# afalchetti/monorfs

Measured on AMD Instinct MI355X. Metric: PHD updates/sec (particles x components x measurements), higher is better.
Workload: dtype f64; 1 GPU; RB-PHD-SLAM SlamUpdate, BASELINE config B: 2048 particles/GPU x 512 components x 64 measurements, PRM3D pixel-range model, prior weights 'survey', state resident in HBM; particles_per_gpu=2048, components=512, measurements=64, max_quantity=600, parallelism=particles sharded x1

## Files before the change

monorfs_amd/csrc/phd_sweep.h:

```cpp
#pragma once
#include "phd_device.h"

#ifndef SW_FIRST1
#define SW_FIRST1 128
#endif
#ifndef SW_TILE1
#define SW_TILE1  128
#endif
#define SW_REC    20
#define SW_UMAX   16

template <int ZB>
struct SweepLds {
	static constexpr int MP = ZB * 64;
	static constexpr int T = (ZB == 1) ? SW_TILE1 : 128;
	static constexpr int NMAP = 256 - T;
	static constexpr int MAPEACH = T / NMAP;
	static_assert(T % 64 == 0 && T < 256 && T % NMAP == 0, "tile: whole waves, and the map-space threads share it evenly");
	static constexpr int TD = (T * SW_REC > MP * 13) ? T * SW_REC : MP * 13;
	static constexpr int zs = 0, zmap = zs + 3 * MP, part = zmap + 3 * MP, part2 = part + 4 * MP, tile = part2 + 4 * MP,
	                     etab = tile + TD, du = etab + EXPTAB_N, ints = du + SW_UMAX;
	static constexpr int doubles = ints + (MP + SW_UMAX + 4) / 2;
};

template <int ZB, bool HALF = false, bool DEPTH = false>
__device__ __forceinline__ void sweep_body(const DevParams& prm, const StepBufs& a, double* pool)
{
	static_assert(!HALF || ZB == 1, "HALF is a layout of the one-block kernel");
	using L = SweepLds<ZB>;
	constexpr int MP = L::MP;
	double* const zs = pool + L::zs;
	double* const zmap = pool + L::zmap;
	double* const part = pool + L::part;
	double* const part2 = pool + L::part2;
	double* const tile = pool + L::tile;
	double* const etab = pool + L::etab;
	double* const s_du = pool + L::du;
	int* const born = (int*) (pool + L::ints);
	int* const s_ulist = born + MP;
	int& s_nb = born[MP + SW_UMAX];
	int& s_nmis = born[MP + SW_UMAX + 1];
	int& s_nu = born[MP + SW_UMAX + 2];

	const int p = a.p0 + blockIdx.x, tid = threadIdx.x, lane = tid & 63, wv = tid >> 6;
	const int M = a.M;
#ifdef PHD_STAMPS
	const long long st_c0 = clock64(), st_r0 = wall_clock64();
	long long st_pairc = 0, st_pairr = 0;
#endif
	const int klane = HALF ? (lane & 31) : lane;
	const int hoff  = HALF ? 4 * (lane >> 5) : 0;
	const bool owner = !HALF || lane < 32;
	const MixView vin = bank_view(a, SEL_IN);
	const Bank bin = bank_of(a, SEL_IN);
	const int n = vin.count[p];
	const size_t sb = in_base(a, p);
	const Bank bout = bank_of(a, SEL_OUT);
	PoseD pose = load_pose(bin.poses + (size_t) p * 7);
	pose.t[0] = uniform_d(pose.t[0]); pose.t[1] = uniform_d(pose.t[1]); pose.t[2] = uniform_d(pose.t[2]);
	pose.qw = uniform_d(pose.qw); pose.qx = uniform_d(pose.qx); pose.qy = uniform_d(pose.qy); pose.qz = uniform_d(pose.qz);
	if (tid < 7) bout.poses[(size_t) p * 7 + tid] = bin.poses[(size_t) p * 7 + tid];
	if (tid == 7) bout.weights[p] = bin.weights[p];
	auto rotation = [&](double* rq) {
		PoseD pq = pose;
		asm volatile("" : "+s"(pq.qw), "+s"(pq.qx), "+s"(pq.qy), "+s"(pq.qz));
		conj_matrix(pq, rq);
	};
	exp_tab_init(etab, tid);
	if (tid == 0) { s_nb = 0; s_nmis = 0; s_nu = 0; }
	for (int k = tid; k < MP; k += 256) {
		double z[3] = {0, 0, 1}, x[3] = {0, 0, 0};
		if (k < M) {
			z[0] = a.z[k * 3]; z[1] = a.z[k * 3 + 1]; z[2] = a.z[k * 3 + 2];
			measure_to_map(prm, pose, z, x);
		}
		zs[k * 3] = z[0]; zs[k * 3 + 1] = z[1]; zs[k * 3 + 2] = z[2];
		zmap[k * 3] = x[0]; zmap[k * 3 + 1] = x[1]; zmap[k * 3 + 2] = x[2];
	}
	__syncthreads();
	double zx[ZB], zy[ZB], zr[ZB], wx[ZB], wy[ZB], wz[ZB], wsum[ZB], dens[ZB];
	bool   zv[ZB];
#pragma unroll
	for (int b = 0; b < ZB; b++) {
		zv[b] = b * 64 + klane < M;
		wsum[b] = 0; dens[b] = 0;
	}
	auto load_z = [&]() {
#pragma unroll
		for (int b = 0; b < ZB; b++) {
			const int k = b * 64 + klane;
			zx[b] = zs[k * 3]; zy[b] = zs[k * 3 + 1]; zr[b] = zs[k * 3 + 2];
			wx[b] = zmap[k * 3]; wy[b] = zmap[k * 3 + 1]; wz[b] = zmap[k * 3 + 2];
		}
	};
	const double g2c = prm.g2_correct, g2e = prm.g2_explore, thr = prm.expl_thr;
	const int segcap = a.candcap >> 2;
	int2* cands = (int2*) a.cand + (size_t) p * a.candcap + (size_t) wv * segcap;
	int ncand_w = 0;

	const double cfac = prm.minw * 0.6065306597126334, ckap = cfac * prm.kappa;
	unsigned long long zvm[ZB];
#pragma unroll
	for (int b = 0; b < ZB; b++) zvm[b] = ballot64(zv[b]);
	const bool allpairs = a.all_pairs != 0;
	auto weigh = [&](const double* tt, int b, double sq, int c, bool cval) {
		const unsigned long long nm = ballot64(sq <= g2c) & (HALF ? ballot64(zv[b] && cval) : zvm[b]);
		if (nm || allpairs) {
			const double x = gauss_logw(tt, zx[b] - tt[0], zy[b] - tt[1], zr[b] - tt[2]);
			const double v = exp_pair(x, etab, zv[b] && sq <= g2c && (!HALF || cval));
			wsum[b] += v;
			const unsigned long long bal = ballot64(v >= fma(cfac, wsum[b], ckap)) & nm;
			if (bal) {
				if ((bal >> lane) & 1ull) {
					const int slot = ncand_w + __popcll(bal & lanemask_lt());
					if (slot < segcap) cands[slot] = make_int2((c << 8) | (b * 64 + klane), __float_as_int((float) x));
				}
				ncand_w += __popcll(bal);
			}
		}
	};

	auto sumk = [&](const double* arr, int k) {
		const double lo = arr[k] + arr[MP + k] + arr[2 * MP + k] + arr[3 * MP + k];
		if (!HALF) return lo;
		return lo + (arr[k + 32] + arr[MP + k + 32] + arr[2 * MP + k + 32] + arr[3 * MP + k + 32]);
	};

	bool compact = false;
	constexpr int SW_TILE = L::T, SW_NMAP = L::NMAP, SW_MAPEACH = L::MAPEACH;
	constexpr int SW_FIRST = (ZB == 1 && SW_FIRST1 < SW_TILE) ? SW_FIRST1 : SW_TILE;
	for (int c0 = 0, tl = SW_FIRST; c0 < n; c0 += tl, tl = SW_TILE) {
		{
			if (tid < SW_NMAP) {
#pragma unroll
				for (int q = 0; q < SW_MAPEACH; q++) {
					const int cl = tid + q * SW_NMAP, c = c0 + cl;
					if (c < n && cl < tl) {
						double P[6], m[3], Pi[6], det, w;
						load_comp(vin.rec + (sb + c) * MIX_REC, w, m, P);
						inv_sym3(P, Pi, det);
						gauss_record(w, m, Pi, PHD_INV_2PI / sqrt(fabs(det)), tile + cl * SW_REC + 10);
					}
				}
			}
			else {
				const int cl = tid - SW_NMAP, c = c0 + cl;
				bool mis = false;
				double wm = 0;
				if (c < n && cl < tl) {
					double* tt = tile + cl * SW_REC;
					double P[6], m[3], w;
					load_comp(vin.rec + (sb + c) * MIX_REC, w, m, P);
					CompMeas q;
					double rq[9];
					rotation(rq);
					comp_measure<DEPTH>(prm, pose, rq, m, P, q);
					tt[0] = q.zh[0]; tt[1] = q.zh[1]; tt[2] = q.zh[2];
					tt[3] = -0.5 * q.Sinv[0];
					tt[4] = -0.5 * (q.Sinv[1] + q.Sinv[3]);
					tt[5] = -0.5 * (q.Sinv[2] + q.Sinv[6]);
					tt[6] = -0.5 * q.Sinv[4];
					tt[7] = -0.5 * (q.Sinv[5] + q.Sinv[7]);
					tt[8] = -0.5 * q.Sinv[8];
					tt[9] = log(q.pd * w * q.qmult);
					wm  = (1 - q.pd) * w;
					mis = !(wm < prm.minw);
				}
				unsigned long long bal = ballot64(mis);
				if (bal) {
					int base = 0, first = __ffsll((long long) bal) - 1;
					if (lane == first) base = atomicAdd(&s_nmis, __popcll(bal));
					base = __shfl(base, first, 64);
					if (mis) {
						int slot = base + __popcll(bal & lanemask_lt());
						if (slot < a.ecap) {
							size_t e = (size_t) p * a.ecap + slot;
							a.emit_w[e]   = wm;
							a.emit_idx[e] = c;
						}
					}
				}
			}
		}
		__syncthreads();
		load_z();
		const int cend = min(tl, n - c0);
		if (compact) {
			const int nu = s_nu;
			for (int u = wv; u < nu; u += 4) {
				const int k = s_ulist[u];
				const double ux = zmap[k * 3], uy = zmap[k * 3 + 1], uz = zmap[k * 3 + 2];
				double acc = 0;
				for (int cc = lane; cc < cend; cc += 64) {
					const double* tt = tile + cc * SW_REC;
					const double e0 = ux - tt[10], e1 = uy - tt[11], e2 = uz - tt[12];
					const double vm = exp_neg(gauss_logw(tt + 10, e0, e1, e2), etab);
					if (e0 * e0 + e1 * e1 + e2 * e2 <= g2e) acc += vm;
				}
#pragma unroll
				for (int o = 32; o > 0; o >>= 1) acc += __shfl_xor(acc, o, 64);
				if (lane == 0) s_du[u] += acc;
			}
		}
		auto visit = [&](int cc) {
			const int ccl = HALF ? min(cc + hoff, cend - 1) : cc;
			const bool cval = !HALF || cc + hoff < cend;
			const double* tt = tile + ccl * SW_REC;
#pragma unroll
			for (int b = 0; b < ZB; b++) {
				double e0 = wx[b] - tt[10], e1 = wy[b] - tt[11], e2 = wz[b] - tt[12];
				double sq = e0 * e0 + e1 * e1 + e2 * e2;
				if (!compact && (allpairs || ballot64(sq <= g2e))) {
					double vm = exp_neg(gauss_logw(tt + 10, e0, e1, e2), etab);
					if (zv[b] && sq <= g2e && cval) dens[b] += vm;
				}
				weigh(tt, b, sq, c0 + ccl, cval);
			}
		};
		int cc = wv;
#ifdef PHD_STAMPS
		const long long st_pc = clock64(), st_pr = wall_clock64();
#endif
		if (HALF) {
			for (; cc < cend; cc += 8) visit(cc);
		}
		else {
			for (; cc + 4 < cend; cc += 8) { visit(cc); visit(cc + 4); }
			if (cc < cend) visit(cc);
		}
#ifdef PHD_STAMPS
		st_pairc += clock64() - st_pc; st_pairr += wall_clock64() - st_pr;
#endif
		if (!compact) {
#pragma unroll
			for (int b = 0; b < ZB; b++) part2[wv * MP + b * 64 + lane] = dens[b];
		}
		__syncthreads();
		if (!compact) {
			int nopen = 0;
			unsigned long long open[ZB];
#pragma unroll
			for (int b = 0; b < ZB; b++) {
				const int k = b * 64 + klane;
				const double d = sumk(part2, k);
				open[b] = ballot64(zv[b] && owner && !(d >= thr));
				nopen += __popcll(open[b]);
			}
			if (nopen <= SW_UMAX) {
				compact = true;
				if (wv == 0) {
					int base = 0;
#pragma unroll
					for (int b = 0; b < ZB; b++) {
						if ((open[b] >> lane) & 1ull) {
							const int u = base + __popcll(open[b] & lanemask_lt());
							s_ulist[u] = b * 64 + lane;
							s_du[u] = 0.0;
						}
						base += __popcll(open[b]);
					}
					if (lane == 0) s_nu = nopen;
				}
			}
		}
	}

#pragma unroll
	for (int b = 0; b < ZB; b++) part2[wv * MP + b * 64 + lane] = dens[b];
	__syncthreads();
	for (int k = tid; k < MP; k += 256) {
		double d = (k < M) ? sumk(part2, k) : 0.0;
		born[k] = (k < M) && !(d >= thr);
	}
	__syncthreads();
	if (tid < s_nu) {
		const int k = s_ulist[tid];
		const double d = sumk(part2, k) + s_du[tid];
		born[k] = !(d >= thr);
	}
	__syncthreads();
	if (tid == 0) {
		int nb = 0;
		for (int k = 0; k < M; k++) {
			if (born[k]) {
				a.born_k[(size_t) p * a.Mcap + nb] = k;
				a.born_mean[((size_t) p * a.Mcap + nb) * 3]     = zmap[k * 3];
				a.born_mean[((size_t) p * a.Mcap + nb) * 3 + 1] = zmap[k * 3 + 1];
				a.born_mean[((size_t) p * a.Mcap + nb) * 3 + 2] = zmap[k * 3 + 2];
				born[nb] = k;
				nb++;
			}
		}
		a.born_count[p] = nb;
		s_nb = nb;
	}
	__syncthreads();
	const int nb = s_nb;
	const int nmis0 = s_nmis;
	__syncthreads();
	if (tid == 0) s_nmis = 0;
	__syncthreads();
	{
		for (int b0 = 0; b0 < nb; b0 += 256) {
			const int bi = b0 + tid;
			bool mis = false;
			double wm = 0, m[3] = {0, 0, 0};
			if (bi < nb) {
				const int k = born[bi];
				m[0] = zmap[k * 3]; m[1] = zmap[k * 3 + 1]; m[2] = zmap[k * 3 + 2];
				CompMeas q;
				double rq[9];
				rotation(rq);
				comp_measure<DEPTH>(prm, pose, rq, m, prm.birthP, q);
				double* tt = tile + bi * 13;
				tt[0] = q.zh[0]; tt[1] = q.zh[1]; tt[2] = q.zh[2];
				tt[3] = -0.5 * q.Sinv[0];
				tt[4] = -0.5 * (q.Sinv[1] + q.Sinv[3]);
				tt[5] = -0.5 * (q.Sinv[2] + q.Sinv[6]);
				tt[6] = -0.5 * q.Sinv[4];
				tt[7] = -0.5 * (q.Sinv[5] + q.Sinv[7]);
				tt[8] = -0.5 * q.Sinv[8];
				tt[9] = log(q.pd * prm.birthw * q.qmult);
				tt[10] = m[0]; tt[11] = m[1]; tt[12] = m[2];
				wm  = (1 - q.pd) * prm.birthw;
				mis = !(wm < prm.minw);
			}
			unsigned long long bal = ballot64(mis);
			if (bal) {
				int base = 0, first = __ffsll((long long) bal) - 1;
				if (lane == first) base = atomicAdd(&s_nmis, __popcll(bal));
				base = __shfl(base, first, 64);
				if (mis) {
					int slot = nmis0 + base + __popcll(bal & lanemask_lt());
					if (slot < a.ecap) {
						size_t e = (size_t) p * a.ecap + slot;
						a.emit_w[e]   = wm;
						a.emit_idx[e] = n + bi;
					}
				}
			}
		}
	}
	__syncthreads();
	load_z();
	for (int bi = (wv - n) & 3; bi < nb; bi += HALF ? 8 : 4) {
		const int bil = HALF ? min(bi + hoff, nb - 1) : bi;
		const bool cval = !HALF || bi + hoff < nb;
		const double* tt = tile + bil * 13;
#pragma unroll
		for (int b = 0; b < ZB; b++) {
			double e0 = wx[b] - tt[10], e1 = wy[b] - tt[11], e2 = wz[b] - tt[12];
			weigh(tt, b, e0 * e0 + e1 * e1 + e2 * e2, n + bil, cval);
		}
	}
#pragma unroll
	for (int b = 0; b < ZB; b++) part[wv * MP + b * 64 + lane] = wsum[b];
	__syncthreads();
	for (int k = tid; k < M; k += 256) {
		a.denom[(size_t) p * a.Mcap + k] = prm.kappa + sumk(part, k);
	}
	if (lane == 0) a.cand_count[(size_t) p * 4 + wv] = ncand_w;
	if (tid == 0) {
		int ne = nmis0 + s_nmis;
		if (ne > a.ecap) { atomicOr(a.flags, PHD_FLAG_EMIT_OVERFLOW); ne = a.ecap; }
		a.emit_count[p] = ne;
	}
#ifdef PHD_STAMPS
	if (tid == 0 && a.stamps && a.stamp_kernel == 6) {
		double* o = a.stamps + (size_t) p * 16;
		o[0] = 0; o[1] = (double) (clock64() - st_c0); o[2] = (double) (wall_clock64() - st_r0); o[3] = (double) st_pairc; o[4] = (double) st_pairr;
	}
#endif
}

#ifndef PHD_SWEEP_WAVES
#define PHD_SWEEP_WAVES 4
#endif
template <int ZB, bool HALF = false, bool DEPTH = false>
#ifndef PHD_SWEEP2_WAVES
#define PHD_SWEEP2_WAVES PHD_SWEEP_WAVES
#endif
__global__ __launch_bounds__(256, (ZB == 4 ? 2 : (ZB == 2 ? PHD_SWEEP2_WAVES : PHD_SWEEP_WAVES))) void k_sweep(const DevParams prm, const StepBufs a)
{
	__shared__ __align__(16) double pool[SweepLds<ZB>::doubles];
	PHD_TL_BEGIN;
	PHD_SET_PRIO(PHD_DENSE_PRIO);
	sweep_body<ZB, HALF, DEPTH>(prm, a, pool);
	PHD_TL_END(6);
}
```

monorfs_amd/csrc/phd_alpha.h:

```cpp
#pragma once
#include "phd_device.h"


__device__ __forceinline__ int pk_get(unsigned int perm, int i) { return (int) ((perm >> (4 * i)) & 15u); }

__device__ __forceinline__ unsigned int pk_set(unsigned int perm, int i, int v)
{
	return (perm & ~(15u << (4 * i))) | ((unsigned int) v << (4 * i));
}

__device__ __forceinline__ unsigned int pk_reverse(unsigned int perm, int from, int to)
{
	for (int i = from, j = to - 1; i < j; i++, j--) {
		int vi = pk_get(perm, i), vj = pk_get(perm, j);
		perm = pk_set(pk_set(perm, i, vj), j, vi);
	}
	return perm;
}

__device__ __forceinline__ bool pk_last(unsigned int perm, int n)
{
	for (int i = 1; i < n; i++) {
		if (pk_get(perm, i - 1) < pk_get(perm, i)) return false;
	}
// ... 682 lines not shown
	__syncthreads();
	const double r = red[0];
	__syncthreads();
	return r;
}

template <int MW>
__device__ __forceinline__ bool has_detection(const unsigned long long* adj, int j)
{
	bool has = false;
#pragma unroll
	for (int b = 0; b < MW; b++) has |= adj[(size_t) j * MW + b] != 0;
	return has;
}

template <int ZB, bool QUASI, bool GRAD = false, int TAG = 0, bool DEPTH = false>
__device__ __forceinline__ void alpha_assoc_body(const DevParams& prm, const StepBufs& a, int ncap, double* smem, double* gws = nullptr,
                                                 int* helper_go = nullptr)
{
	constexpr int MP = ZB * 64;
	constexpr int MW = ZB;
	constexpr int JL = ALPHA_JL;
	const AlphaLds lay = alpha_lds(MP, ncap);
	double* zs   = smem + lay.zs;
	double* red  = smem + lay.red;
	double* etab = red;
	__shared__ int s_J, s_changed[2], s_nroots, s_big;
	__shared__ double s_ccount, s_total;
	__shared__ int s_ebump, s_g2lds;
	__shared__ double s_g2[GRAD ? QGRAD_G2_CLUSTERS * QGRAD_HDR + QGRAD_G2_WEIGHTS : 2];
	if (GRAD && threadIdx.x == 0) s_g2lds = 0;

	const int p = a.p0 + blockIdx.x, tid = threadIdx.x, lane = tid & 63, wv = tid >> 6;
	const int M = a.M, cap = a.cap;
	const MixView vout = bank_view(a, SEL_OUT);
	const Bank bin = bank_of(a, SEL_IN);
	const int no = QUASI ? 0 : vout.count[p];
	const size_t sbo = (size_t) p * cap;
	const PoseD pose = load_pose(QUASI ? a.qposes + (size_t) p * 7 : bin.poses + (size_t) p * 7);

	for (int k = tid; k < MP * 3; k += 256) zs[k] = (k < M * 3) ? a.z[k] : 0.0;
	unsigned int helper_word = 0;
	if (!QUASI && helper_go && tid == 0) helper_word = __hip_atomic_load(a.dsync + 3 * (size_t) p, __ATOMIC_RELAXED, __HIP_MEMORY_SCOPE_AGENT);

	PHD_STAMP_DECL;
	PHD_STAMP(0);
	double* keyw    = smem + lay.p1_keyw;
	double* sortw   = smem + lay.p1_sortw;
	int*    sortsrc = (int*) (smem + lay.p1_sortsrc);
	auto block_sum = [&](double v) { return block_tree_sum(red, v, tid); };
	double wpart = 0;
	for (int c = tid; c < no; c += 256) {
		double wc = a.outw[sbo + c];
		keyw[c] = wc;
		wpart += wc;
	}
	{
		double e = block_sum(wpart);
		if (fabs(e - rint(e)) <= 1e-9 * fmax(1.0, fabs(e))) {
			if (tid == 0) {
				double q = 0;
				for (int c = 0; c < no; c++) q += keyw[c];
				s_ccount = q;
			}
			__syncthreads();
			e = s_ccount;
		}
		if (tid == 0) {
			s_ccount = e;
			int J = (int) e;
			if (J < 0) J = 0;
			if (J > a.Jcap) {
				atomicOr(a.flags, PHD_FLAG_J_OVERFLOW);
				J = a.Jcap;
			}
			s_J = QUASI ? min(a.qJ, a.Jcap) : J;
		}
	}
	PHD_STAMP(1);
	__syncthreads();
	const int J = s_J;
	if (J >= 1 && J <= no) {
		constexpr int HB = 500;
		int* const hist   = (int*) red;
		int* const selidx = (int*) (smem + lay.p1_selidx);
		int* const pre    = (int*) (smem + lay.p1_dw);
		int& s_T = hist[HB];
		int& s_above = hist[HB + 1];
		int& s_nt = hist[HB + 2];
		const unsigned int hbase = (unsigned int) (((unsigned long long) __double_as_longlong(prm.minw) << 1) >> 49);
		auto bin_of = [&](double w) {
			const unsigned int k = (unsigned int) (((unsigned long long) __double_as_longlong(w) << 1) >> 49);
			return (int) min(max((int) k - (int) hbase, 0), HB - 1);
		};
		for (int t = tid; t < HB + 4; t += 256) hist[t] = 0;
		__syncthreads();
		for (int c = tid; c < no; c += 256) atomicAdd(&hist[bin_of(keyw[c])], 1);
		__syncthreads();
		if (wv == 0) {
			int cq[8], mine = 0;
#pragma unroll
			for (int q = 0; q < 8; q++) { const int b = 511 - (8 * lane + q); cq[q] = (b < HB) ? hist[b] : 0; mine += cq[q]; }
			int incl = mine;
#pragma unroll
			for (int o = 1; o < 64; o <<= 1) {
				const int y = __shfl_up(incl, o, 64);
				if (lane >= o) incl += y;
			}
			int run = incl - mine;
#pragma unroll
			for (int q = 0; q < 8; q++) {
				const int b = 511 - (8 * lane + q);
				if (b < HB) pre[b] = run;
				if (run < J && J <= run + cq[q]) { s_T = b; s_above = run; s_nt = cq[q]; }
				run += cq[q];
			}
		}
		__syncthreads();
		const int T = s_T, above = s_above;
		const int ncand = above + s_nt;
		for (int c = tid; c < no; c += 256) {
			const int b = bin_of(keyw[c]);
			if (b >= T) selidx[pre[b] + atomicSub(&hist[b], 1) - 1] = c;
		}
		__syncthreads();
		for (int e = tid; e < ncand; e += 256) {
			const int ce = selidx[e];
			const double we = keyw[ce];
			const int b = bin_of(we);
			const int lo = pre[b], hi = (b == T) ? ncand : pre[b - 1];
			int rank = lo;
#pragma unroll 4
			for (int u = lo; u < hi; u++) {
				const int cu = selidx[u];
				const double wu = keyw[cu];
				rank += (wu > we || (wu == we && cu < ce)) ? 1 : 0;
			}
			if (rank < J) { sortw[rank] = we; sortsrc[rank] = ce; }
		}
		__syncthreads();
	}
	else if (!QUASI && J > no) {
		unsigned long long* sv = (unsigned long long*) sortw;
		int NS = 2;
		while (NS < no) NS <<= 1;
		for (int t = tid; t < NS; t += 256) sv[t] = (t < no) ? prune_pack(keyw[t], t) : 0ull;
		__syncthreads();
		prune_bitonic(sv, NS, tid);
		for (int r = tid; r + 1 < no; r += 256) {
			const unsigned long long kb = prune_kbits(sv[r]);
			if (prune_kbits(sv[r + 1]) != kb || (r > 0 && prune_kbits(sv[r - 1]) == kb)) continue;
			int e = r + 2;
			while (e < no && prune_kbits(sv[e]) == kb) e++;
			for (int x = r + 1; x < e; x++) {
				unsigned long long vx = sv[x];
				int sx = prune_slot(vx);
				double wx = keyw[sx];
				int y = x - 1;
				while (y >= r) {
					int sy = prune_slot(sv[y]);
					if (keyw[sy] > wx || (keyw[sy] == wx && sy < sx)) break;
					sv[y + 1] = sv[y];
					y--;
				}
				sv[y + 1] = vx;
			}
		}
		__syncthreads();
		for (int r = tid; r < no; r += 256) sortsrc[r] = prune_slot(sv[r]);
		__syncthreads();
		for (int r = tid; r < no; r += 256) sortw[r] = keyw[sortsrc[r]];
		__syncthreads();
	}
	PHD_STAMP(2);
	const bool inlds = J <= JL;
	const int  JS = inlds ? JL : a.Jcap;
	double* gj = a.jscratch + (size_t) p * alpha_jscratch_doubles(a.Jcap);
	double* lm   = inlds ? smem + lay.lm     : gj + AlphaSlab::lm * (size_t) JS;
	double* dw   = inlds ? smem + lay.p1_dw  : gj + AlphaSlab::dw * (size_t) JS;
	double* zh   = inlds ? smem + lay.p3_zh  : gj + AlphaSlab::zh * (size_t) JS;
	double* lpd  = inlds ? smem + lay.p3_pdj : gj + AlphaSlab::lpd * (size_t) JS;
	double* lmd  = inlds ? smem + lay.p3_lmd : gj + AlphaSlab::lmd * (size_t) JS;
	double* res  = inlds ? smem + lay.p3_res : gj + AlphaSlab::res * (size_t) JS;
	unsigned long long* adj = (unsigned long long*) (inlds ? smem + lay.p3_adj : gj + AlphaSlab::adj * (size_t) JS);
	int* gi      = (int*) (gj + AlphaSlab::ints * (size_t) JS);
	int* pick    = inlds ? (int*) (smem + lay.pick) : gi + AlphaSlab::i_pick * JS;
	int* dsrc    = inlds ? sortsrc + lay.ns : gi + AlphaSlab::i_dsrc * JS;
	int* labl    = inlds ? (int*) (smem + lay.p3_int) : gi + AlphaSlab::i_labl * JS;
	int* roots   = inlds ? labl + JL : gi + AlphaSlab::i_roots * JS;
	int* cnt     = inlds ? labl + 2 * JL : (int*) (gj + AlphaSlab::cnt * (size_t) JS);
	unsigned long long* memL = (unsigned long long*) (inlds ? smem + lay.p3_mem : gj + AlphaSlab::memL * (size_t) JS);
	unsigned long long* memZ = (unsigned long long*) (inlds ? smem + lay.p3_mem + JL : gj + AlphaSlab::memZ * (size_t) JS);
	int* labz    = (int*) (smem + lay.p3_int) + 3 * JL;
	double* xreg = smem + lay.p3_x;
	const bool straight = J <= no && (J == 0 || !(sortw[0] - 1 > sortw[J - 1]));
	if (QUASI) {}
	else if (straight) {
		for (int j = tid; j < J; j += 256) pick[j] = sortsrc[j];
	}
	else if (tid == 0) {
		int ia = 0, id = 0, nd = 0;
		for (int j = 0; j < J; j++) {
			bool takeorig;
			if (ia < no && id < nd) takeorig = !(dw[id] > sortw[ia]);
			else takeorig = ia < no;
			double wpick;
			int    src;
			if (takeorig) { wpick = sortw[ia]; src = sortsrc[ia]; ia++; }
			else          { wpick = dw[id];    src = dsrc[id];    id++; }
			dw[nd]   = wpick - 1;
			dsrc[nd] = src;
			nd++;
			pick[j] = src;
		}
	}
	__threadfence_block();
	__syncthreads();
	constexpr int JW = JL / 64;
	unsigned long long* adjT = (unsigned long long*) (smem + lay.p3_adjT);
	for (int k = tid; k < M; k += 256) labz[k] = J + k;
	for (int t = tid; t < MP * JW; t += 256) adjT[t] = 0;
	if (tid == 0) { s_nroots = 0; s_big = 0; s_changed[0] = 0; }
	for (int j = tid; j < J; j += 256) {
		double2 r0 = {0.0, 0.0}, r1 = {0.0, 0.0};
		if (!QUASI) {
			const double2* rc = (const double2*) (vout.rec + (sbo + pick[j]) * MIX_REC);
			r0 = rc[0]; r1 = rc[1];
		}
#pragma unroll
		for (int b = 0; b < MW; b++) adj[(size_t) j * MW + b] = 0;
		labl[j] = j;
		cnt[j]  = 0;
		memL[j] = 0;
		memZ[j] = 0;
		if (QUASI) {
			lm[j] = a.qlm[j * 3]; lm[JS + j] = a.qlm[j * 3 + 1]; lm[2 * JS + j] = a.qlm[j * 3 + 2];
		}
		else {
			double l0 = r0.y, l1 = r1.x, l2 = r1.y;
			lm[j] = l0; lm[JS + j] = l1; lm[2 * JS + j] = l2;
			double* glm = a.alm + (size_t) p * 3 * a.Jcap;
			glm[j] = l0; glm[a.Jcap + j] = l1; glm[2 * a.Jcap + j] = l2;
		}
	}
	if (!QUASI && helper_go) {
		if (tid == 0) { a.aJ[p] = J; a.account[p] = s_ccount; }
		asm volatile("s_waitcnt vmcnt(0)" ::: "memory");
	}
	__threadfence_block();
	__syncthreads();
	if (!QUASI && helper_go && tid == 0) {
		const int go = (dens_layout(J) != DensLayout::slab && helper_word == ((a.dstamp << 4) | my_xcd())) ? 1 : 0;
		__hip_atomic_store(a.dsync + 3 * (size_t) p + 1, 2u * a.dstamp + (unsigned int) go, __ATOMIC_RELAXED, __HIP_MEMORY_SCOPE_AGENT);
		*helper_go = go;
#ifdef PHD_STAMPS
		if (a.stamps && a.stamp_kernel == 5) { a.stamps[(size_t) p * 16 + 12] = go; a.stamps[(size_t) p * 16 + 13] = (double) wall_clock64(); }
#endif
	}

	PHD_STAMP(3);
	{
		double* mats = xreg;

		const bool pair = J <= 128;
		for (int t = tid; t < (pair ? 256 : J); t += 256) {
			const int j = pair ? (t & 127) : t;
			if (j >= J) continue;
			double m[3] = {lm[j], lm[JS + j], lm[2 * JS + j]}, z[3], l[3];
			measure_perfect(prm, pose, m, z, l);
			const float dz = (!QUASI && DEPTH) ? depth_at(prm, z) : 0.0f;
			const double pdv = QUASI ? prm.pd : detection_probability_m<!QUASI && DEPTH>(prm, z, dz);
			if (!pair || t < 128) {
				zh[j] = z[0]; zh[JS + j] = z[1]; zh[2 * JS + j] = z[2];
				lpd[j] = log(pdv);
			}
			if (!pair || t >= 128) lmd[j] = log(1 - pdv);
		}
		__threadfence_block();
		__syncthreads();
		{
			double kx[ZB], ky[ZB], kz[ZB];
#pragma unroll
			for (int b = 0; b < ZB; b++) {
				const int k = b * 64 + lane;
				kx[b] = zs[k * 3]; ky[b] = zs[k * 3 + 1]; kz[b] = zs[k * 3 + 2];
			}
			const double g2 = QUASI ? prm.g2_quasi : prm.g2_assoc;
			for (int j = wv; j < J; j += 4) {
				const double h0 = zh[j], h1 = zh[JS + j], h2 = zh[2 * JS + j];
#pragma unroll
				for (int b = 0; b < ZB; b++) {
					const int k = b * 64 + lane;
					const bool gated = k < M && quad_gen(prm.Rinv, h0 - kx[b], h1 - ky[b], h2 - kz[b]) < g2;
					const unsigned long long bal = ballot64(gated);
					if (lane == 0) adj[(size_t) j * MW + b] = bal;
					if (gated && inlds) atomicOr(&adjT[(size_t) k * JW + (j >> 6)], 1ull << (j & 63));
				}
			}
		}
		__threadfence_block();
		__syncthreads();

		PHD_STAMP(4);
		for (int it = 0; it < J + M + 1; it++) {
			int* const changed = &s_changed[it & 1];
			for (int j = tid; j < J; j += 256) {
				int l = labl[j];
#pragma unroll
				for (int b = 0; b < MW; b++) {
					unsigned long long bits = adj[(size_t) j * MW + b];
					while (bits) {
						int k = b * 64 + __ffsll((long long) bits) - 1;
						bits &= bits - 1;
						l = min(l, labz[k]);
					}
				}
				if (l < labl[j]) { labl[j] = l; *changed = 1; }
			}
			__threadfence_block();
			__syncthreads();
			if (tid == 0) s_changed[(it & 1) ^ 1] = 0;
			for (int k = tid; k < M; k += 256) {
				int l = labz[k];
				if (inlds) {
#pragma unroll
					for (int b = 0; b < JW; b++) {
						unsigned long long bits = adjT[(size_t) k * JW + b];
						while (bits) {
							int j = b * 64 + __ffsll((long long) bits) - 1;
							bits &= bits - 1;
							l = min(l, labl[j]);
						}
					}
				}
				else {
					for (int j = 0; j < J; j++) {
						if ((adj[(size_t) j * MW + (k >> 6)] >> (k & 63)) & 1ull) l = min(l, labl[j]);
					}
				}
				if (l < labz[k]) { labz[k] = l; *changed = 1; }
			}
			__threadfence_block();
			__syncthreads();
			if (!*changed) break;
		}
		for (int j = tid; j < J; j += 256) {
			const int r = labl[j];
			const int slot = atomicAdd(&cnt[r], 1) & 0xffff;
			if (slot < 5) atomicOr(&memL[r], (unsigned long long) j << (12 * slot));
		}
		for (int k = tid; k < M; k += 256) {
			const int r = labz[k];
			if (r < J) {
				const int slot = atomicAdd(&cnt[r], 0x10000) >> 16;
				if (slot < 5) atomicOr(&memZ[r], (unsigned long long) k << (12 * slot));
			}
		}
		if (wv == 0) {
			int nr = 0;
			for (int j0 = 0; j0 < J; j0 += 64) {
				const int j = j0 + lane;
				bool isroot = false;
				if (j < J) {
					const bool has = has_detection<MW>(adj, j);
					isroot = has && labl[j] == j;
				}
				unsigned long long bal = ballot64(isroot);
				if (isroot) roots[nr + __popcll(bal & lanemask_lt())] = j;
				nr += __popcll(bal);
			}
			if (lane == 0) s_nroots = nr;
		}
		exp_tab_init(etab, tid);
		__syncthreads();
		const int nroots = s_nroots;
		const double logmult = prm.logRmult;

		PHD_STAMP(5);
		if (GRAD) {
			if (tid == 0) s_big = 1;
		}
		else if (J >= 5) {
			for (int ri = tid; ri < nroots; ri += 256) {
				const int root = roots[ri];
				const int cn = cnt[root];
				const int nl = cn & 0xffff, nz = cn >> 16;
				if (nl + nz > 5) {
					res[ri] = NAN;
					s_big = 1;
					continue;
				}
				const unsigned long long Lp = pk_sort5(memL[root], nl), Zp = pk_sort5(memZ[root], nz);
				double E[25];
#pragma unroll
				for (int e = 0; e < 25; e++) E[e] = (e % 6 == 0) ? 1.0 : 0.0;
				double rsum = 0;
				bool dead = false;
#pragma unroll
				for (int x = 0; x < 4; x++) {
					if (x < nl) {
						const int j = (int) ((Lp >> (12 * x)) & 4095);
						const double md = lmd[j], lp = lpd[j];
						const double h0 = zh[j], h1 = zh[JS + j], h2 = zh[2 * JS + j];
						double D[4], rx = md;
#pragma unroll
						for (int y = 0; y < 4 - x; y++) {
							D[y] = -INFINITY;
							if (y < nz) {
								const int k = (int) ((Zp >> (12 * y)) & 4095);
								if ((adj[(size_t) j * MW + (k >> 6)] >> (k & 63)) & 1ull) {
									double dist = sqrt(quad_gen(prm.Rinv, h0 - zs[k * 3], h1 - zs[k * 3 + 1], h2 - zs[k * 3 + 2]));
									D[y] = lp + logmult - 0.5 * dist * dist;
									rx = fmax(rx, D[y]);
								}
							}
						}
						if (rx == -INFINITY) dead = true;
						else {
							rsum += rx;
							E[x * 6] = exp_neg(md - rx, etab);
#pragma unroll
							for (int y = 0; y < 4 - x; y++) {
								if (y < nz) E[x * 5 + 4 - y] = (D[y] == -INFINITY) ? 0.0 : exp_neg(D[y] - rx, etab);
							}
						}
					}
				}
#pragma unroll
				for (int y = 0; y < 4; y++) {
					if (y < nz) {
						E[(4 - y) * 6] = prm.kappa;
#pragma unroll
						for (int x = 0; x < 4 - y; x++) {
							if (x < nl) E[(4 - y) * 5 + x] = 1.0;
						}
					}
				}
				double f[32];
#pragma unroll
				for (int m = 0; m < 32; m++) f[m] = 0;
				f[0] = 1;
#pragma unroll
				for (int i = 0; i < 5; i++) {
#pragma unroll
					for (int m = 0; m < 32; m++) {
						if (__builtin_popcount(m) == i) {
#pragma unroll
							for (int c = 0; c < 5; c++) {
								if (!((m >> c) & 1)) f[m | (1 << c)] = fma(f[m], E[i * 5 + c], f[m | (1 << c)]);
							}
						}
					}
				}
				res[ri] = dead ? -INFINITY : rsum + log(f[31]);
			}
		}
		else if (wv == 0) {
			for (int r0 = 0; r0 < nroots; r0 += 64) {
				int ri = r0 + lane;
				if (ri < nroots) {
					int root = roots[ri];
					unsigned long long Lp = 0, Zp = 0;
					int nl = 0, nz = 0, nrow = 0;
					for (int j = root; j < J; j++) {
						if (labl[j] == root) { if (nl < 5) Lp |= (unsigned long long) j << (12 * nl); nl++; }
					}
					for (int k = 0; k < M; k++) {
						if (labz[k] == root) { if (nz < 5) Zp |= (unsigned long long) k << (12 * nz); nz++; }
					}
					nrow = nl + nz;
					if (nrow > 5) {
						res[ri] = NAN;
						s_big = 1;
					}
					else {
						double* mat = mats + lane;
						for (int e = 0; e < 25; e++) mat[e * 4] = -INFINITY;
						for (int x = 0; x < nl; x++) {
							int j = (int) ((Lp >> (12 * x)) & 4095);
							for (int y = 0; y < nz; y++) {
								int k = (int) ((Zp >> (12 * y)) & 4095);
								if ((adj[(size_t) j * MW + (k >> 6)] >> (k & 63)) & 1ull) {
									double dist = sqrt(quad_gen(prm.Rinv, zh[j] - zs[k * 3], zh[JS + j] - zs[k * 3 + 1],
									                            zh[2 * JS + j] - zs[k * 3 + 2]));
									mat[(x * 5 + y) * 4] = lpd[j] + logmult - 0.5 * dist * dist;
								}
							}
							mat[(x * 5 + nz + x) * 4] = lmd[j];
						}
						for (int y = 0; y < nz; y++) {
							mat[((nl + y) * 5 + y) * 4] = prm.logkappa;
							for (int x = 0; x < nl; x++) mat[((nl + y) * 5 + nz + x) * 4] = 0;
						}
						res[ri] = cluster_enumerate(mat, 4, nrow, J);
					}
				}
			}
		}
		__syncthreads();
		if (GRAD && gws && inlds) {
			double* const wsm = gws + wv * QGRAD_WAVE_DOUBLES;
			double* const gmat = wsm;
			double* const gjp = wsm + 25;
			double (*gdv)[6] = (double (*)[6]) (wsm + 25 + 5 * 18);
			double* const glc = wsm + 25 + 5 * 18 + 120 * 6;
			int* const gL = (int*) (glc + 120);
			int* const gZ = gL + 8;
			double* const jpall = gj + AlphaSlab::g_jpall;
			double* const elist = gj + AlphaSlab::g_elist;
			const int ecap = (int) alpha_jscratch_doubles(a.Jcap) - AlphaSlab::g_elist;
			const int gt = (lane < 6) ? lane : 0;
			if (tid == 0) s_ebump = 0;
			if (ecap > 0) {
				for (int j = tid; j < J; j += 256) {
					const double m3[3] = {lm[j], lm[JS + j], lm[2 * JS + j]};
					jacobian_p(prm, pose, m3, jpall + (size_t) j * 18);
				}
			}
			__threadfence_block();
			__syncthreads();
			const bool pairfast = J >= 5 && ecap > 0;
			if (pairfast) {
				for (int ri = tid; ri < nroots; ri += 256) {
					const int root = roots[ri];
					if (cnt[root] != 0x10001) continue;
					const int j = (int) (memL[root] & 4095), k = (int) (memZ[root] & 4095);
					double* const h = gj + (size_t) ri * QGRAD_HDR;
					const bool gated = (adj[(size_t) j * MW + (k >> 6)] >> (k & 63)) & 1ull;
					double c0 = -INFINITY;
					if (gated) {
						double dist = sqrt(quad_gen(prm.Rinv, zh[j] - zs[k * 3], zh[JS + j] - zs[k * 3 + 1], zh[2 * JS + j] - zs[k * 3 + 2]));
						c0 = lpd[j] + logmult - 0.5 * dist * dist;
					}
					c0 = (0.0 + c0) + 0.0;
					const double c1 = (0.0 + lmd[j]) + prm.logkappa;
					const double mx = fmax(fmax(-INFINITY, c0), c1);
					const bool finite = !(isinf(mx) && mx < 0);
					double lse = -INFINITY, w0 = c0, w1 = c1;
					if (finite) {
						double value = 0;
						value += exp(c0 - mx);
						value += exp(c1 - mx);
						lse = mx + log(value);
						w0 = exp_neg(c0 - mx, etab);
						w1 = exp_neg(c1 - mx, etab);
					}
					res[ri] = lse;
					const int off = atomicAdd(&s_ebump, 2);
					if (off + 2 > ecap) { h[0] = -2; continue; }
					elist[off] = w0;
					elist[off + 1] = w1;
					double G[6] = {0, 0, 0, 0, 0, 0};
					if (finite && gated) {
						const double nu[3] = {zs[k * 3] - zh[j], zs[k * 3 + 1] - zh[JS + j], zs[k * 3 + 2] - zh[2 * JS + j]};
						const double* Jp = jpall + (size_t) j * 18;
#pragma unroll
						for (int t = 0; t < 6; t++) G[t] = w0 * (0.0 + pair_gradient(prm, nu, Jp, t));
					}
					h[0] = 2.0;
#pragma unroll
					for (int t = 0; t < 6; t++) h[1 + t] = G[t];
					h[7] = (double) off;
					h[8] = finite ? 1.0 : 0.0;
				}
			}
			PHD_STAMP(9);
			for (int ri = wv; ri < nroots; ri += 4) {
				const int root = roots[ri];
				if (pairfast && cnt[root] == 0x10001) continue;
				double* const h = gj + (size_t) ri * QGRAD_HDR;
				int nl = 0, nz = 0;
				for (int j0 = root; j0 < J; j0 += 64) {
					const int j = j0 + lane;
					const bool in = j < J && labl[j] == root;
					const unsigned long long bal = ballot64(in);
					const int pos = nl + __popcll(bal & lanemask_lt());
					if (in && pos < 6) gL[pos] = j;
					nl += __popcll(bal);
				}
				for (int k0 = 0; k0 < M; k0 += 64) {
					const int k = k0 + lane;
					const bool in = k < M && labz[k] == root;
					const unsigned long long bal = ballot64(in);
					const int pos = nz + __popcll(bal & lanemask_lt());
					if (in && pos < 6) gZ[pos] = k;
					nz += __popcll(bal);
				}
				const int nrow = nl + nz;
				if (nrow > 5) {
					if (lane == 0) h[0] = -1;
					continue;
				}
				lds_fence();
				if (lane < nrow * nrow) {
					const int x = lane / nrow, y = lane - x * nrow;
					double v = -INFINITY;
					if (x < nl) {
						const int j = gL[x];
						if (y < nz) {
							const int k = gZ[y];
							if ((adj[(size_t) j * MW + (k >> 6)] >> (k & 63)) & 1ull) {
								double dist = sqrt(quad_gen(prm.Rinv, zh[j] - zs[k * 3], zh[JS + j] - zs[k * 3 + 1], zh[2 * JS + j] - zs[k * 3 + 2]));
								v = lpd[j] + logmult - 0.5 * dist * dist;
							}
						}
						else if (y - nz == x) v = lmd[j];
					}
					else {
						if (y < nz) { if (y == x - nl) v = prm.logkappa; }
						else v = 0;
					}
					gmat[x * 5 + y] = v;
				}
				if (ecap <= 0) {
					if (lane == 0) h[0] = -2;
					continue;
				}
				int mcount;
				double mx = -INFINITY, value = 0;
				if (nrow <= J) {
					double* const pgt = gjp;
					const int npair = nl * nz;
					bool g = false;
					{
						const int pr = lane / 6, t = lane - 6 * pr;
						if (pr < npair) {
							const int x = pr / nz, y = pr - x * nz;
							const int j = gL[x], k = gZ[y];
							g = (adj[(size_t) j * MW + (k >> 6)] >> (k & 63)) & 1ull;
							double v = 0;
							if (g) {
								const double nu[3] = {zs[k * 3] - zh[j], zs[k * 3 + 1] - zh[JS + j], zs[k * 3 + 2] - zh[2 * JS + j]};
								v = pair_gradient(prm, nu, jpall + (size_t) j * 18, t);
							}
							pgt[(x * 4 + y) * 6 + t] = v;
						}
					}
					const unsigned long long gb = ballot64(g);
					unsigned int gmask = 0;
					for (int pr = 0; pr < npair; pr++) {
						if ((gb >> (6 * pr)) & 1ull) gmask |= 1u << ((pr / nz) * 4 + (pr % nz));
					}
					lds_fence();
					mcount = 1;
					for (int i = 2; i <= nrow; i++) mcount *= i;
					double vv[2] = {-INFINITY, -INFINITY};
#pragma unroll
					for (int pass = 0; pass < 2; pass++) {
						const int m = lane + 64 * pass;
						if (m < mcount) {
							const unsigned int perm = pk_unrank(m, nrow);
							double v = 0;
							for (int i = 0; i < nrow; i++) v += gmat[i * 5 + pk_get(perm, i)];
							double acc[6] = {0, 0, 0, 0, 0, 0};
							for (int x = 0; x < nl; x++) {
								const int y = pk_get(perm, x);
								if (y < nz && ((gmask >> (x * 4 + y)) & 1u)) {
#pragma unroll
									for (int t = 0; t < 6; t++) acc[t] += pgt[(x * 4 + y) * 6 + t];
								}
							}
							glc[m] = v;
#pragma unroll
							for (int t = 0; t < 6; t++) gdv[m][t] = acc[t];
							vv[pass] = v;
						}
					}
					mx = fmax(vv[0], vv[1]);
#pragma unroll
					for (int o = 32; o > 0; o >>= 1) mx = fmax(mx, __shfl_xor(mx, o, 64));
					if (!(isinf(mx) && mx < 0)) {
						const double e0 = (lane < mcount) ? exp(vv[0] - mx) : 0.0, e1 = (lane + 64 < mcount) ? exp(vv[1] - mx) : 0.0;
						auto rld = [](double v, int l) {
							return __hiloint2double(__builtin_amdgcn_readlane(__double2hiint(v), l), __builtin_amdgcn_readlane(__double2loint(v), l));
						};
						for (int i = 0; i < mcount; i++) value += (i < 64) ? rld(e0, i) : rld(e1, i - 64);
// ... 863 lines not shown
```

Before: 125.3 billion PHD updates/s.

## Build sweep birth list with wave ballots and drop serial scan and barriers

After: 125.9 billion PHD updates/s (median of 6 runs). About the same (+0.5%).

```diff
diff --git a/monorfs_amd/csrc/phd_sweep.h b/monorfs_amd/csrc/phd_sweep.h
--- a/monorfs_amd/csrc/phd_sweep.h
+++ b/monorfs_amd/csrc/phd_sweep.h
@@ -22,6 +22,8 @@
 	                     etab = tile + TD, du = etab + EXPTAB_N, ints = du + SW_UMAX;
 	static constexpr int doubles = ints + (MP + SW_UMAX + 4) / 2;
 };
+static_assert(SweepLds<1>::doubles * 8 <= 32768 && 4 * SweepLds<2>::doubles * 8 <= 160 * 1024,
+              "k_sweep<1> and k_sweep<2> run four workgroups per CU: their LDS must fit 160 KiB four times");
 
 template <int ZB, bool HALF = false, bool DEPTH = false>
 __device__ __forceinline__ void sweep_body(const DevParams& prm, const StepBufs& a, double* pool)
@@ -47,6 +49,8 @@
 #ifdef PHD_STAMPS
 	const long long st_c0 = clock64(), st_r0 = wall_clock64();
 	long long st_pairc = 0, st_pairr = 0;
+	long long st_tail = st_c0, st_list = 0, st_stage = 0;
+	int st_switch = -1, st_tile = 0;
 #endif
 	const int klane = HALF ? (lane & 31) : lane;
 	const int hoff  = HALF ? 4 * (lane >> 5) : 0;
@@ -65,6 +69,23 @@
 		PoseD pq = pose;
 		asm volatile("" : "+s"(pq.qw), "+s"(pq.qx), "+s"(pq.qy), "+s"(pq.qz));
 		conj_matrix(pq, rq);
+	};
+	auto birth_record = [&](int k, double* tt) {
+		const double m[3] = {zmap[k * 3], zmap[k * 3 + 1], zmap[k * 3 + 2]};
+		CompMeas q;
+		double rq[9];
+		rotation(rq);
+		comp_measure<DEPTH>(prm, pose, rq, m, prm.birthP, q);
+		tt[0] = q.zh[0]; tt[1] = q.zh[1]; tt[2] = q.zh[2];
+		tt[3] = -0.5 * q.Sinv[0];
+		tt[4] = -0.5 * (q.Sinv[1] + q.Sinv[3]);
+		tt[5] = -0.5 * (q.Sinv[2] + q.Sinv[6]);
+		tt[6] = -0.5 * q.Sinv[4];
+		tt[7] = -0.5 * (q.Sinv[5] + q.Sinv[7]);
+		tt[8] = -0.5 * q.Sinv[8];
+		tt[9] = log(q.pd * prm.birthw * q.qmult);
+		tt[10] = m[0]; tt[11] = m[1]; tt[12] = m[2];
+		return (1 - q.pd) * prm.birthw;
 	};
 	exp_tab_init(etab, tid);
 	if (tid == 0) { s_nb = 0; s_nmis = 0; s_nu = 0; }
@@ -230,6 +251,7 @@
 		}
 #ifdef PHD_STAMPS
 		st_pairc += clock64() - st_pc; st_pairr += wall_clock64() - st_pr;
+		st_tail = clock64();
 #endif
 		if (!compact) {
 #pragma unroll
@@ -248,6 +270,9 @@
 			}
 			if (nopen <= SW_UMAX) {
 				compact = true;
+#ifdef PHD_STAMPS
+				st_switch = st_tile;
+#endif
 				if (wv == 0) {
 					int base = 0;
 #pragma unroll
@@ -263,66 +288,78 @@
 				}
 			}
 		}
-	}
-
-#pragma unroll
-	for (int b = 0; b < ZB; b++) part2[wv * MP + b * 64 + lane] = dens[b];
+#ifdef PHD_STAMPS
+		st_tile++;
+#endif
+	}
+
+	if (n == 0) {
+#pragma unroll
+		for (int b = 0; b < ZB; b++) part2[wv * MP + b * 64 + lane] = dens[b];
+		__syncthreads();
+	}
+#ifdef PHD_STAMPS
+	st_list = clock64();
+#endif
+	if (wv == 0) {
+		int nbw = 0;
+		auto list = [&](bool isb, int k, int bi) {
+			if (isb) {
+				a.born_k[(size_t) p * a.Mcap + bi] = k;
+				a.born_mean[((size_t) p * a.Mcap + bi) * 3]     = zmap[k * 3];
+				a.born_mean[((size_t) p * a.Mcap + bi) * 3 + 1] = zmap[k * 3 + 1];
+				a.born_mean[((size_t) p * a.Mcap + bi) * 3 + 2] = zmap[k * 3 + 2];
+				born[bi] = k;
+			}
+		};
+		if (compact) {
+			const int nu = s_nu;
+			bool isb = false;
+			int k = 0;
+			if (lane < nu) {
+				k = s_ulist[lane];
+				const double d = sumk(part2, k) + s_du[lane];
+				isb = !(d >= thr);
+			}
+			const unsigned long long bal = ballot64(isb);
+			const int bi = __popcll(bal & lanemask_lt());
+			nbw = __popcll(bal);
+			list(isb, k, bi);
+		}
+		else {
+			bool isb[ZB];
+			unsigned long long bal[ZB];
+#pragma unroll
+			for (int b = 0; b < ZB; b++) {
+				const int k = b * 64 + lane;
+				const double d = (k < M) ? sumk(part2, k) : 0.0;
+				isb[b] = (k < M) && !(d >= thr);
+				bal[b] = ballot64(isb[b]);
+			}
+#pragma unroll
+			for (int b = 0; b < ZB; b++) {
+				list(isb[b], b * 64 + lane, nbw + __popcll(bal[b] & lanemask_lt()));
+				nbw += __popcll(bal[b]);
+			}
+		}
+		if (lane == 0) {
+			a.born_count[p] = nbw;
+			s_nb = nbw;
+		}
+	}
 	__syncthreads();
-	for (int k = tid; k < MP; k += 256) {
-		double d = (k < M) ? sumk(part2, k) : 0.0;
-		born[k] = (k < M) && !(d >= thr);
-	}
-	__syncthreads();
-	if (tid < s_nu) {
-		const int k = s_ulist[tid];
-		const double d = sumk(part2, k) + s_du[tid];
-		born[k] = !(d >= thr);
-	}
-	__syncthreads();
-	if (tid == 0) {
-		int nb = 0;
-		for (int k = 0; k < M; k++) {
-			if (born[k]) {
-				a.born_k[(size_t) p * a.Mcap + nb] = k;
-				a.born_mean[((size_t) p * a.Mcap + nb) * 3]     = zmap[k * 3];
-				a.born_mean[((size_t) p * a.Mcap + nb) * 3 + 1] = zmap[k * 3 + 1];
-				a.born_mean[((size_t) p * a.Mcap + nb) * 3 + 2] = zmap[k * 3 + 2];
-				born[nb] = k;
-				nb++;
-			}
-		}
-		a.born_count[p] = nb;
-		s_nb = nb;
-	}
-	__syncthreads();
-	const int nb = s_nb;
-	const int nmis0 = s_nmis;
-	__syncthreads();
-	if (tid == 0) s_nmis = 0;
-	__syncthreads();
-	{
+#ifdef PHD_STAMPS
+	st_stage = clock64();
+	st_list = st_stage - st_list;
+#endif
+	const int nb = __builtin_amdgcn_readfirstlane(s_nb);
+	if (nb > 0) {
 		for (int b0 = 0; b0 < nb; b0 += 256) {
 			const int bi = b0 + tid;
 			bool mis = false;
-			double wm = 0, m[3] = {0, 0, 0};
+			double wm = 0;
 			if (bi < nb) {
-				const int k = born[bi];
-				m[0] = zmap[k * 3]; m[1] = zmap[k * 3 + 1]; m[2] = zmap[k * 3 + 2];
-				CompMeas q;
-				double rq[9];
-				rotation(rq);
-				comp_measure<DEPTH>(prm, pose, rq, m, prm.birthP, q);
-				double* tt = tile + bi * 13;
-				tt[0] = q.zh[0]; tt[1] = q.zh[1]; tt[2] = q.zh[2];
-				tt[3] = -0.5 * q.Sinv[0];
-				tt[4] = -0.5 * (q.Sinv[1] + q.Sinv[3]);
-				tt[5] = -0.5 * (q.Sinv[2] + q.Sinv[6]);
-				tt[6] = -0.5 * q.Sinv[4];
-				tt[7] = -0.5 * (q.Sinv[5] + q.Sinv[7]);
-				tt[8] = -0.5 * q.Sinv[8];
-				tt[9] = log(q.pd * prm.birthw * q.qmult);
-				tt[10] = m[0]; tt[11] = m[1]; tt[12] = m[2];
-				wm  = (1 - q.pd) * prm.birthw;
+				wm  = birth_record(born[bi], tile + bi * 13);
 				mis = !(wm < prm.minw);
 			}
 			unsigned long long bal = ballot64(mis);
@@ -331,7 +368,7 @@
 				if (lane == first) base = atomicAdd(&s_nmis, __popcll(bal));
 				base = __shfl(base, first, 64);
 				if (mis) {
-					int slot = nmis0 + base + __popcll(bal & lanemask_lt());
+					int slot = base + __popcll(bal & lanemask_lt());
 					if (slot < a.ecap) {
 						size_t e = (size_t) p * a.ecap + slot;
 						a.emit_w[e]   = wm;
@@ -340,8 +377,11 @@
 				}
 			}
 		}
-	}
-	__syncthreads();
+		__syncthreads();
+	}
+#ifdef PHD_STAMPS
+	st_stage = clock64() - st_stage;
+#endif
 	load_z();
 	for (int bi = (wv - n) & 3; bi < nb; bi += HALF ? 8 : 4) {
 		const int bil = HALF ? min(bi + hoff, nb - 1) : bi;
@@ -361,7 +401,7 @@
 	}
 	if (lane == 0) a.cand_count[(size_t) p * 4 + wv] = ncand_w;
 	if (tid == 0) {
-		int ne = nmis0 + s_nmis;
+		int ne = s_nmis;
 		if (ne > a.ecap) { atomicOr(a.flags, PHD_FLAG_EMIT_OVERFLOW); ne = a.ecap; }
 		a.emit_count[p] = ne;
 	}
@@ -369,6 +409,8 @@
 	if (tid == 0 && a.stamps && a.stamp_kernel == 6) {
 		double* o = a.stamps + (size_t) p * 16;
 		o[0] = 0; o[1] = (double) (clock64() - st_c0); o[2] = (double) (wall_clock64() - st_r0); o[3] = (double) st_pairc; o[4] = (double) st_pairr;
+		o[5] = (double) (clock64() - st_tail); o[6] = (double) st_list; o[7] = (double) st_stage;
+		o[8] = nb; o[9] = s_nu; o[10] = st_switch;
 	}
 #endif
 }
```

## Run connected-component label propagation in a single wavefront when measurements fit one wave

Applied to the files above, without the earlier changes.

Result: no change. 125.8 billion PHD updates/s before, 125.8 billion PHD updates/s after (-0.0%).

```diff
diff --git a/monorfs_amd/csrc/phd_alpha.h b/monorfs_amd/csrc/phd_alpha.h
--- a/monorfs_amd/csrc/phd_alpha.h
+++ b/monorfs_amd/csrc/phd_alpha.h
@@ -1008,7 +1008,38 @@
 		__syncthreads();
 
 		PHD_STAMP(4);
-		for (int it = 0; it < J + M + 1; it++) {
+		const bool onewave = ZB == 1 && pair && M <= 64;
+		if (onewave && wv == 0) {
+			const int ja = lane, jb = lane + 64, k = lane;
+			const unsigned long long ea = (ja < J) ? adj[(size_t) ja * MW] : 0ull, eb = (jb < J) ? adj[(size_t) jb * MW] : 0ull;
+			const unsigned long long t0 = (k < M) ? adjT[(size_t) k * JW] : 0ull, t1 = (k < M) ? adjT[(size_t) k * JW + 1] : 0ull;
+			int la = ja, lb = jb, lz = J + k;
+			auto least = [](unsigned long long bits, const int* lab, int l) {
+				while (bits) {
+					l = min(l, lab[__ffsll((long long) bits) - 1]);
+					bits &= bits - 1;
+				}
+				return l;
+			};
+			for (;;) {
+				const int na = least(ea, labz, la), nb = least(eb, labz, lb);
+				bool ch = na < la || nb < lb;
+				if (na < la) labl[ja] = la = na;
+				if (nb < lb) labl[jb] = lb = nb;
+				lds_fence();
+				__builtin_amdgcn_wave_barrier();
+				const int nz = least(t1, labl + 64, least(t0, labl, lz));
+				ch |= nz < lz;
+				if (nz < lz) labz[k] = lz = nz;
+				lds_fence();
+				__builtin_amdgcn_wave_barrier();
+				if (!ballot64(ch)) break;
+			}
+		}
+		else if (onewave) {
+			for (int t = tid - 64; t < EXPTAB_N; t += 192) etab[t] = exp2((double) t / EXPTAB_N);
+		}
+		for (int it = 0; it < J + M + 1 && !onewave; it++) {
 			int* const changed = &s_changed[it & 1];
 			for (int j = tid; j < J; j += 256) {
 				int l = labl[j];
@@ -1050,12 +1081,13 @@
 			__syncthreads();
 			if (!*changed) break;
 		}
-		for (int j = tid; j < J; j += 256) {
+		const int mt0 = onewave ? (wv == 0 ? lane : J + M) : tid, mts = onewave ? 64 : 256;
+		for (int j = mt0; j < J; j += mts) {
 			const int r = labl[j];
 			const int slot = atomicAdd(&cnt[r], 1) & 0xffff;
 			if (slot < 5) atomicOr(&memL[r], (unsigned long long) j << (12 * slot));
 		}
-		for (int k = tid; k < M; k += 256) {
+		for (int k = mt0; k < M; k += mts) {
 			const int r = labz[k];
 			if (r < J) {
 				const int slot = atomicAdd(&cnt[r], 0x10000) >> 16;
@@ -1077,7 +1109,7 @@
 			}
 			if (lane == 0) s_nroots = nr;
 		}
-		exp_tab_init(etab, tid);
+		if (!onewave) exp_tab_init(etab, tid);
 		__syncthreads();
 		const int nroots = s_nroots;
 		const double logmult = prm.logRmult;
```
